# wnmusic/simpleFE

Hardware: AMD Instinct MI355X
Metric: complex-float32 MS/s through 256-tap blkconv FIR; % of HBM roofline (higher is better)
Workload: dtype f32

## Files before the change

simplefe_amd/build.py:

```python
import glob
import json
import os
import subprocess
import sys

HERE = os.path.dirname(os.path.abspath(__file__))
CSRC = os.path.join(HERE, "csrc")
LIB = os.path.join(HERE, "libsfe_dsp.so")
LIB_DIAG = os.path.join(HERE, "libsfe_dsp_diag.so")
ARCH = "gfx950"
EXACT_SOURCES = ("polyphase.hip", "util.hip", "chan.hip", "combine.hip", "ddc.hip")
TICKET_SOURCES = ("fir_fft.hip", "poly_fft.hip")
HOST_SOURCES = ("api.hip", "api_plans.hip", "api_fir.hip", "api_rs.hip", "api_pipe.hip", "api_chan.hip", "api_combine.hip", "api_ddc.hip",
                "group.hip", "host.h")


def sources(diag=False):
    return sorted(glob.glob(os.path.join(CSRC, "*.hip"))) + (sorted(glob.glob(os.path.join(CSRC, "diag", "*.hip"))) if diag else [])


def _deps():
    return sources(diag=True) + glob.glob(os.path.join(CSRC, "*.h")) + glob.glob(os.path.join(CSRC, "diag", "*.inc")) + glob.glob(
        os.path.join(os.path.dirname(HERE), "include", "*.h"))


KERNEL_FILES = {"fir": ("fir_fft.hip", "fft16.h", "common.h"), "resample": ("poly_fft.hip", "fft16.h", "common.h"),
                "decimate": ("polyphase.hip", "common.h"), "chan": ("chan.hip", "fft16.h", "common.h"),
                "combine": ("combine.hip", "fft16.h", "common.h"), "ddc": ("ddc.hip", "common.h")}


def csrc_hash(kind=None):
    import hashlib
    import re
    h = hashlib.sha256()
    paths = sorted(glob.glob(os.path.join(CSRC, "*.hip")) + glob.glob(os.path.join(CSRC, "*.h")))
    if kind is not None:
        paths = [p for p in paths if os.path.basename(p) in KERNEL_FILES[kind]]
    for p in paths:
        if os.path.basename(p) in HOST_SOURCES:
            continue
        h.update(os.path.basename(p).encode() + b"\0")
        depth, skip_at = 0, None
        for line in open(p, errors="replace"):
            code = re.sub(r"\s+", " ", re.sub(r"//.*$", "", line)).strip()
            if code.startswith("#if"):
                depth += 1
                if skip_at is None and re.match(r"#ifdef SFE_DIAG\b", code):
                    skip_at = depth
                    continue
            elif code.startswith("#else") and skip_at == depth:
                skip_at = -depth
                continue
            elif code.startswith("#endif"):
                closing = depth
                depth -= 1
                if skip_at is not None and abs(skip_at) == closing:
                    skip_at = None
                    continue
            if skip_at is not None and skip_at > 0:
                continue
            if code:
                h.update(code.encode() + b"\n")
        h.update(b"\0")
    return h.hexdigest()


def needs_build(lib=LIB):
    if not os.path.exists(lib):
        return True
    t = os.path.getmtime(lib)
    return any(os.path.getmtime(p) > t for p in _deps())


def parse_resources(text):
    import re
    out, cur = {}, None
    for line in text.splitlines():
        m = re.search(r"remark:\s+Function Name: (\S+)", line)
        if m:
            cur = out.setdefault(m.group(1), {})
            continue
        m = re.search(r"remark:\s+(TotalSGPRs|VGPRs|AGPRs|ScratchSize \[bytes/lane\]|Occupancy \[waves/SIMD\]|SGPRs Spill|VGPRs Spill|"
                      r"LDS Size \[bytes/block\]): (\d+)", line)
        if m and cur is not None:
            cur[m.group(1).split(" [")[0]] = int(m.group(2))
    if out:
        names = list(out)
        try:
            dem = subprocess.run(["c++filt"], input="\n".join(names), capture_output=True, text=True).stdout.splitlines()
        except OSError:
            dem = []
        if len(dem) == len(names):
            out = {d: out[n] for d, n in zip(dem, names)}
    return out


FIR_TEMPLATE_ARGS = "IN_C OUT_C IN_U8 PAIR OUT_TX10 DMA DIAG ACC WP HCH".split()


def fir_kernel_flags(name):
    import re
    m = re.search(r"fir_fft4096_kernel<(.*?)>\(", name)
    if not m:
        return None
    vals = [a.strip() for a in m.group(1).split(",")]
    return {k: (v == "true" if v in ("true", "false") else int(v)) for k, v in zip(FIR_TEMPLATE_ARGS, vals)}


def check_resources(res):
# ... 83 lines not shown
```

simplefe_amd/csrc/diag/fir_fft_diag.inc:

```
template <int WAVES>
__global__ __launch_bounds__(256, WAVES) void fir_copy_pattern_kernel(FirFftArgs a)
{
    const unsigned t = threadIdx.x;
    const char *in_c = static_cast<const char *>(a.in) + (size_t)blockIdx.y * a.in_stride * 8;
    char *out_c = static_cast<char *>(a.out) + (size_t)blockIdx.y * a.out_stride * 8;
    const int row0 = a.hl >> 8;
    for (long long blk = blockIdx.x; blk < a.nblk; blk += gridDim.x) {
        const long long base = blk * a.advance - a.hl;
        if (base < 0 || base + FFT_N > a.n) continue;
        v2f v[16];
#pragma unroll
        for (int r = 0; r < 16; r++) v[r] = load_sample<true>(in_c + (base + 256 * r) * 8, t);
#pragma unroll
        for (int r = 0; r < 16; r++)
            if (r >= row0) reinterpret_cast<v2f *>(out_c + (base + 256 * r) * 8)[t] = v[r];
    }
}


template <int WAVES>
__global__ __launch_bounds__(256, WAVES) void fir_copy_pattern16_kernel(FirFftArgs a)
{
    const unsigned t = threadIdx.x;
    const char *in_c = static_cast<const char *>(a.in) + (size_t)blockIdx.y * a.in_stride * 8;
    char *out_c = static_cast<char *>(a.out) + (size_t)blockIdx.y * a.out_stride * 8;
    const int row0 = a.hl >> 8;
    const unsigned half = t >> 7, col2 = t & 127;
    for (long long blk = blockIdx.x; blk < a.nblk; blk += gridDim.x) {
        const long long base = blk * a.advance - a.hl;
        if (base < 0 || base + FFT_N > a.n) continue;
        v4f v[8];
#pragma unroll
        for (int j = 0; j < 8; j++)
            v[j] = reinterpret_cast<const v4f *>(in_c + (base + 256 * (2 * j)) * 8)[col2 + 128 * half];
#pragma unroll
        for (int j = 0; j < 8; j++)
            if (2 * j + (int)half >= row0)
                reinterpret_cast<v4f *>(out_c + (base + 256 * (2 * j)) * 8)[col2 + 128 * half] = v[j];
    }
}

#define FIR_TRACE_WGS 163840
__device__ unsigned long long g_fir_trace[5 * FIR_TRACE_WGS];
__device__ unsigned long long g_fir_tdone[FIR_TRACE_WGS];
__device__ unsigned long long g_fir_tclk[FIR_TRACE_WGS];
__device__ int g_fir_gate;
__device__ int g_fir_order;

template <int WAVES, bool TICKET, bool BAR = false, bool TRACE = false>
__global__ __launch_bounds__(256, WAVES) void fir_copy_pattern_nt_kernel(FirFftArgs a)
{
    __shared__ unsigned s_next;
    const unsigned t = threadIdx.x;
    const unsigned long long t_start = TRACE ? wall_clock64() : 0ull;
    const int gate = TRACE ? g_fir_gate : 0;
    const int order = TRACE ? g_fir_order : 0;
    unsigned n_done = 0;
    const unsigned wg_lin = blockIdx.x + blockIdx.y * gridDim.x;
    auto leave = [&]() {
        if (TRACE && t == 0 && wg_lin < FIR_TRACE_WGS) {
            unsigned long long *r = g_fir_trace + 5ull * wg_lin;
            r[0] = t_start; r[1] = wall_clock64(); r[2] = n_done;
            r[3] = __builtin_amdgcn_s_getreg(20 | (3 << 11));
            r[4] = __builtin_amdgcn_s_getreg(4 | (31 << 11));
        }
    };
    const int row0 = a.hl >> 8;
    const unsigned nblk32 = (unsigned)a.nblk;
    const unsigned tg = a.tgroups, grp = blockIdx.x % tg;
    unsigned *const my_ticket = a.ticket + 32u * grp;
    const unsigned last_draw = (a.total > grp ? (a.total - grp + tg - 1u) / tg : 0u) + (gridDim.x - grp + tg - 1u) / tg - 1u;
    auto draw = [&]() -> unsigned {
        const unsigned c = __hip_atomic_fetch_add(my_ticket, 1u, __ATOMIC_RELAXED, __HIP_MEMORY_SCOPE_AGENT);
        if (c == last_draw) __hip_atomic_store(my_ticket, 0u, __ATOMIC_RELAXED, __HIP_MEMORY_SCOPE_AGENT);
        const unsigned long long k = (unsigned long long)c * tg + grp;
        return k < a.total ? (unsigned)k : 0xFFFFFFFFu;
    };
    unsigned kt = 0;
    long long blk = blockIdx.x;
    int ch = TICKET ? 0 : blockIdx.y;
    if (TICKET) {
        if (t == 0) s_next = draw();
        lds_barrier();
        kt = __builtin_amdgcn_readfirstlane(s_next);
        lds_barrier();
    }
    for (;;) {
        if (TICKET) {
            if (kt >= a.total) break;
            ch = (int)(kt / nblk32);
            blk = kt - (unsigned)ch * nblk32;
        } else if (blk >= a.nblk) break;
        const char *in_c = static_cast<const char *>(a.in) + (size_t)ch * a.in_stride * 8;
        char *out_c = static_cast<char *>(a.out) + (size_t)ch * a.out_stride * 8;
        long long pblk = blk;
        if (order == 1) pblk = a.nblk - 1 - blk;
        else if (order == 2) pblk = (long long)(((unsigned long long)blk * 48271ull) % (unsigned long long)a.nblk);
        const long long base = pblk * a.advance - a.hl;
        unsigned drawn = 0;
        if (TICKET && t == 0) drawn = draw();
        if (base >= 0 && base + FFT_N <= a.n) {
            v2f v[16];
            if (gate) while (((wall_clock64() >> gate) & 1ull) != 0ull) __builtin_amdgcn_s_sleep(1);
#pragma unroll
            for (int r = 0; r < 16; r++)
                v[r] = __builtin_nontemporal_load(reinterpret_cast<const v2f *>(in_c + (base + 256 * r) * 8) + t);
            if (BAR) { asm volatile("s_waitcnt vmcnt(0)" ::: "memory"); lds_barrier(); lds_barrier(); }
            if (gate) {
                asm volatile("s_waitcnt vmcnt(0)" ::: "memory");
                while (((wall_clock64() >> gate) & 1ull) != 1ull) __builtin_amdgcn_s_sleep(1);
            }
#pragma unroll
            for (int r = 0; r < 16; r++)
                if (r >= row0) __builtin_nontemporal_store(v[r], reinterpret_cast<v2f *>(out_c + (base + 256 * r) * 8) + t);
            if (TRACE && t == 0 && v[15].x != 1.2345e38f) {
                const unsigned long long lin = (unsigned long long)ch * nblk32 + (unsigned long long)blk;
                if (lin < FIR_TRACE_WGS) { g_fir_tdone[lin] = wall_clock64(); g_fir_tclk[lin] = clock64(); }
            }
        }
        n_done++;
        if (TICKET) {
            if (t == 0) s_next = drawn;
            lds_barrier();
            kt = __builtin_amdgcn_readfirstlane(s_next);
            lds_barrier();
        } else blk += gridDim.x;
// ... 153 lines not shown
```

simplefe_amd/csrc/diag/fir_fft_launch_diag.inc:

```
    if (ev && in_complex && out_complex && !in_u8 && !out_tx10) {
#define SFE_NEW(DM, DG, WPV) SFE_K(true, true, false, false, false, DM, DG, false, WPV)
#define SFE_NEW_DG(DM, WPV) do { if (diag == 1) SFE_NEW(DM, 1, WPV); else if (diag == 2) SFE_NEW(DM, 2, WPV); \
                                else if (diag == 3) SFE_NEW(DM, 3, WPV); else SFE_NEW(DM, 0, WPV); } while (0)
        bool done = true;
        const bool traced = (ev[0] == 'e' || ev[0] == 'E') && (getenv("SFE_FIR_TRACE") || getenv("SFE_FIR_ORDER") || getenv("SFE_FIR_GATE"));
        if (traced) {
            const int order = getenv("SFE_FIR_ORDER") ? atoi(getenv("SFE_FIR_ORDER")) : 0;
            SFE_HIP(hipMemcpyToSymbolAsync(HIP_SYMBOL(g_fir_order), &order, sizeof order, 0, hipMemcpyHostToDevice, s));
            const int gate = getenv("SFE_FIR_GATE") ? atoi(getenv("SFE_FIR_GATE")) : 0;
            SFE_HIP(hipMemcpyToSymbolAsync(HIP_SYMBOL(g_fir_gate), &gate, sizeof gate, 0, hipMemcpyHostToDevice, s));
        }
        if (ev[0] == 'c') hipLaunchKernelGGL((fir_copy_pattern_kernel<4>), grid2, block, 0, s, a);
        else if (ev[0] == 'd') hipLaunchKernelGGL((fir_copy_pattern16_kernel<4>), grid2, block, 0, s, a);
        else if (ev[0] == 'e' && traced) hipLaunchKernelGGL((fir_copy_pattern_nt_kernel<4, false, false, true>), grid2, block, 0, s, a);
        else if (ev[0] == 'E' && traced) hipLaunchKernelGGL((fir_copy_pattern_nt_kernel<4, true, false, true>), grid, block, 0, s, a);
        else if (ev[0] == 'e') hipLaunchKernelGGL((fir_copy_pattern_nt_kernel<4, false>), grid2, block, 0, s, a);
        else if (ev[0] == 'E') hipLaunchKernelGGL((fir_copy_pattern_nt_kernel<4, true>), grid, block, 0, s, a);
        else if (ev[0] == 'b') hipLaunchKernelGGL((fir_copy_pattern_nt_kernel<4, false, true>), grid2, block, 0, s, a);
        else if (ev[0] == 'g') hipLaunchKernelGGL((fir_copy_pattern_dma_kernel<4, true>), grid2, block, 0, s, a);
        else if (ev[0] == 'G') hipLaunchKernelGGL((fir_copy_pattern_dma_kernel<4, false>), grid2, block, 0, s, a);
        else if (ev[0] == 'q' || ev[0] == 'Q') {
            const int delay = getenv("SFE_FIR_DELAY") ? atoi(getenv("SFE_FIR_DELAY")) : 0;
            SFE_HIP(hipMemcpyToSymbolAsync(HIP_SYMBOL(g_fir_delay), &delay, sizeof delay, 0, hipMemcpyHostToDevice, s));
            if (ev[0] == 'q') hipLaunchKernelGGL((fir_copy_pattern_dma2_kernel<2, true>), grid2, block, 0, s, a);
            else hipLaunchKernelGGL((fir_copy_pattern_dma2_kernel<4, false>), grid2, block, 0, s, a);
        }
        else if (ev[0] == 'p') hipLaunchKernelGGL((fir_copy_pattern_pipe_kernel<4>), grid2, block, 0, s, a);
        else if (ev[0] == 'T') SFE_NEW_DG(false, false);
        else if (ev[0] == 'X') SFE_NEW_DG(true, false);
        else if (ev[0] == 'W') SFE_NEW_DG(true, true);
        else if (ev[0] == 'y') SFE_NEW(true, 8, false);
        else if (ev[0] == 'u') SFE_NEW(false, 8, false);
        else if (ev[0] == 'L') SFE_NEW(false, 16, false);
        else if (ev[0] == 'M') SFE_NEW(false, 32, false);
        else if (ev[0] == 'N') SFE_NEW(false, 48, false);
        else if (ev[0] == 'l') SFE_NEW(true, 16, false);
        else if (ev[0] == 'n') SFE_NEW(true, 48, false);
        else if (ev[0] == 'x') SFE_NEW(true, 4, false);
        else if (ev[0] == 't') SFE_NEW(false, 4, false);
        else if (ev[0] == 'w') SFE_NEW(true, 4, true);
        else done = false;
#undef SFE_NEW
#undef SFE_NEW_DG
        if (done) {
            SFE_HIP(hipGetLastError());
            if (const char *tp = getenv("SFE_FIR_TRACE")) {
                if (traced) {
                    const size_t nwg = (ev[0] == 'E' ? (size_t)grid.x : (size_t)grid2.x * grid2.y);
                    const size_t cnt = 5 * (nwg < FIR_TRACE_WGS ? nwg : FIR_TRACE_WGS);
                    unsigned long long *h = (unsigned long long *)malloc(cnt * 8);
                    SFE_HIP(hipStreamSynchronize(s));
                    SFE_HIP(hipMemcpyFromSymbol(h, HIP_SYMBOL(g_fir_trace), cnt * 8));
                    if (FILE *f = fopen(tp, "wb")) { fwrite(h, 8, cnt, f); fclose(f); }
                    free(h);
                    const size_t nt = a.total < FIR_TRACE_WGS ? a.total : FIR_TRACE_WGS;
                    h = (unsigned long long *)malloc(nt * 8);
                    SFE_HIP(hipMemcpyFromSymbol(h, HIP_SYMBOL(g_fir_tdone), nt * 8));
                    char tp2[512];
                    snprintf(tp2, sizeof tp2, "%s.done", tp);
                    if (FILE *f = fopen(tp2, "wb")) { fwrite(h, 8, nt, f); fclose(f); }
                    SFE_HIP(hipMemcpyFromSymbol(h, HIP_SYMBOL(g_fir_tclk), nt * 8));
                    snprintf(tp2, sizeof tp2, "%s.clk", tp);
                    if (FILE *f = fopen(tp2, "wb")) { fwrite(h, 8, nt, f); fclose(f); }
                    free(h);
                }
            }
            return SFE_OK;
        }
    }
```

simplefe_amd/csrc/fir_fft.hip:

```cpp
#include <stdint.h>
#include <stdlib.h>

#include "common.h"
#include "fft16.h"

namespace sfe {
namespace {

template <bool IN_C, bool IN_U8 = false>
__device__ __forceinline__ v2f load_sample(const void *p, unsigned lane)
{
    if constexpr (IN_U8) {
        if constexpr (IN_C) {
            const unsigned w = __builtin_nontemporal_load(reinterpret_cast<const unsigned short *>(p) + lane);
            return (v2f){u8_to_f32(w & 0xFFu), u8_to_f32(w >> 8)};
        } else {
            return (v2f){u8_to_f32(__builtin_nontemporal_load(reinterpret_cast<const unsigned char *>(p) + lane)), 0.0f};
        }
    }
    if constexpr (IN_C) return __builtin_nontemporal_load(reinterpret_cast<const v2f *>(p) + lane);
    else return (v2f){__builtin_nontemporal_load(reinterpret_cast<const float *>(p) + lane), 0.0f};
}

template <int K>
__device__ __forceinline__ unsigned quad_lane(unsigned v)
{
    return (unsigned)__builtin_amdgcn_update_dpp(0, (int)v, K | (K << 2) | (K << 4) | (K << 6), 0xF, 0xF, true);
}
__device__ __forceinline__ unsigned quad_odd(unsigned v)
{
    return (unsigned)__builtin_amdgcn_update_dpp(0, (int)v, 1 | (1 << 2) | (3 << 4) | (3 << 6), 0xF, 0xF, true);
}

__device__ __forceinline__ void store_group(unsigned char *d, unsigned u0, unsigned u1, unsigned u2, unsigned u3)
{
    const unsigned w = ((u0 >> 8) | ((u1 >> 8) << 2) | ((u2 >> 8) << 4) | ((u3 >> 8) << 6)) | ((u0 & 0xFFu) << 8) |
                       ((u1 & 0xFFu) << 16) | ((u2 & 0xFFu) << 24);
    __builtin_memcpy(d, &w, 4);
    d[4] = (unsigned char)u3;
}

#ifdef SFE_DIAG
__device__ unsigned long long g_fir_clk[4];
#define SFE_FIR_STAMP(i)                                                                   \
    do {                                                                                   \
        if (blockIdx.x == 0 && blockIdx.y == 0 && threadIdx.x == 0) {                      \
            g_fir_clk[i] = __builtin_amdgcn_s_memtime();                                   \
            g_fir_clk[(i) + 1] = __builtin_amdgcn_s_memrealtime();                         \
        }                                                                                  \
    } while (0)
#else
#define SFE_FIR_STAMP(i) do { } while (0)
#endif

template <bool IN_C, bool OUT_C, bool IN_U8 = false, bool PAIR = false, bool OUT_TX10 = false, bool DMA = false, int DIAG = 0,
          bool ACC = false, bool WP = false, bool HCH = false>
__global__ __launch_bounds__(256, 4) void fir_fft4096_kernel(FirFftArgs a)
{
    static_assert(!WP || DMA, "the wave-private layout exists for the LDS-DMA path");
    static_assert(!ACC || (!OUT_TX10 && !DMA), "accumulating launches write float32 through the plain store path");
    static_assert(!DMA || (IN_C && !IN_U8 && !PAIR), "LDS-DMA input: complex float32, padded layout");
    constexpr bool INTERLEAVE = (DIAG & 8) != 0;
    constexpr bool NOMID = (DIAG & 16) != 0, NORECON = (DIAG & 32) != 0;
    auto tw2f = [](v2f x, v2f q, v2f p) -> v2f { return NORECON ? cmul(x, q) : cmul2(x, q, p); };
    auto tw2i = [](v2f x, v2f q, v2f p) -> v2f { return NORECON ? cmul_conj(x, q) : cmul2_conj(x, q, p); };
    __shared__ v2f lds[WP ? 4 * WP_REGION : FFT_ROWS * LDS_K2_STRIDE];
    __shared__ unsigned s_next;
    const unsigned t = threadIdx.x;
    SFE_FIR_STAMP(0);
    int ch = 0;
    const unsigned lo = t & 15, hi = t >> 4;
    const unsigned base_a = WP ? (t >> 6) * WP_REGION + (t & 63u) : t;
    const unsigned base_b = hi * LDS_K2_STRIDE + lo;
    const unsigned base_c = hi * LDS_K2_STRIDE + lo * LDS_K1_STRIDE;
    const unsigned base_w = (hi & 7u) * WP_PITCH + (hi >> 3) * 64u + lo;
    auto row_a = [](int r) -> unsigned { return WP ? (unsigned)((r & 7) * WP_PITCH + (r >> 3) * 64) : (unsigned)(r * LDS_K2_STRIDE); };
    auto cell_b1 = [&](int a1) -> unsigned {
        if (WP) return base_w + (unsigned)((a1 >> 2) * WP_REGION + 16 * (a1 & 3));
        return base_b + 16u * a1;
    };
    auto cell_b2 = [&](int a1) -> unsigned { return base_b + (unsigned)LDS_K1_STRIDE * a1; };
    auto cell_c = [&](int n0) -> unsigned { return base_c + n0; };

    constexpr int ISZ = IN_U8 ? (IN_C ? 2 : 1) : (IN_C ? 8 : 4);
    const char *in_c, *hist_c;
    char *out_c;
    auto in_of = [&](int c) -> const char * { return static_cast<const char *>(a.in) + (size_t)c * a.in_stride * ISZ; };
    v2f hreg[16];
    auto load_spectrum = [&](int c) {
        if constexpr (HCH) {
#pragma unroll
            for (int k = 0; k < 16; k++) {
                hreg[k] = (a.hs + (size_t)c * a.hs_stride + k * 256)[threadIdx.x];
                asm volatile("" : "+v"(hreg[k]));
            }
        }
    };
    auto set_channel = [&](int c) {
        in_c = in_of(c);
        out_c = static_cast<char *>(a.out) + (OUT_TX10 ? (size_t)c * (a.out_stride * (OUT_C ? 2 : 1) / 4) * 5 : (size_t)c * a.out_stride * (OUT_C ? 8 : 4));
        hist_c = static_cast<const char *>(a.hist) + (size_t)c * a.hist_len * (IN_C ? 8 : 4);
    };
    load_spectrum(ch);
    set_channel(ch);

    v2f p1[4], q1[4], p2[4], q2[4];
#pragma unroll
    for (int k = 1; k < 4; k++) {
        p1[k] = a.tw1[k * 256 + t];
        q1[k] = a.tw1[(k + 3) * 256 + t];
        p2[k] = a.tw2[k * 16 + lo];
        q2[k] = a.tw2[(k + 3) * 16 + lo];
    }

    const int row0 = a.hl >> 8;
    auto carry_history = [&]() {
        char *ho = static_cast<char *>(a.hist_out) + (size_t)ch * a.hist_len * (IN_C ? 8 : 4);
        for (int r = 0; r < (a.hist_len >> 8); r++) {
            const v2f s = load_sample<IN_C, IN_U8>(in_c + (a.n - a.hist_len + 256 * r) * ISZ, t);
            if constexpr (IN_C) reinterpret_cast<v2f *>(ho)[256 * r + t] = s;
            else reinterpret_cast<float *>(ho)[256 * r + t] = s.x;
        }
    };
    const unsigned tg = a.tgroups, grp = blockIdx.x % tg;
    unsigned *const my_ticket = a.ticket + 32u * grp;
    const unsigned Q = 1u << a.tqs, row = tg << a.tqs, rem = a.total % row;
    const bool by_channel = HCH && a.ch_groups;
    const unsigned mine = by_channel ? (a.total / (unsigned)a.nblk / tg) * (unsigned)a.nblk
                                     : (a.total / row << a.tqs) + (rem > grp * Q ? (rem - grp * Q < Q ? rem - grp * Q : Q) : 0u);
    const unsigned last_draw = mine + (gridDim.x - grp + tg - 1u) / tg - 1u;
    const bool few = a.total <= gridDim.x;
    auto draw_issue = [&]() -> unsigned {
        if (few) return 0u;
        return __hip_atomic_fetch_add(my_ticket, 1u, __ATOMIC_RELAXED, __HIP_MEMORY_SCOPE_AGENT);
    };
    auto draw_finish = [&](unsigned c) -> unsigned {
        if (few) return 0xFFFFFFFFu;
        if (c == last_draw) __hip_atomic_store(my_ticket, 0u, __ATOMIC_RELAXED, __HIP_MEMORY_SCOPE_AGENT);
        if (by_channel) {
            if (c >= mine) return 0xFFFFFFFFu;
            const unsigned i = c / (unsigned)a.nblk;
            return (grp + tg * i) * (unsigned)a.nblk + (c - i * (unsigned)a.nblk);
        }
        const unsigned long long k = (((unsigned long long)(c >> a.tqs) * tg + grp) << a.tqs) + (c & (Q - 1u));
        return k < a.total ? (unsigned)k : 0xFFFFFFFFu;
    };
    auto draw = [&]() -> unsigned { return draw_finish(draw_issue()); };
    const unsigned nblk32 = (unsigned)a.nblk;
    if (!HCH) {
#pragma unroll
        for (int k = 0; k < 16; k++) {
            hreg[k] = (a.hs + k * 256)[t];
            asm volatile("" : "+v"(hreg[k]));
        }
    }

    auto load_rows = [&](v2f (&x)[16], long long blk) {
        constexpr int ESZ = IN_C ? 8 : 4;
        if constexpr (PAIR) {
            const long long baseA = 2 * blk * a.advance - a.hl - a.shift, baseB = baseA + a.advance;
            if constexpr (IN_U8) {
                if (baseA >= 0 && baseB + FFT_N <= a.n && (reinterpret_cast<uintptr_t>(in_c) & 15u) == 0) {
                    typedef unsigned v4u __attribute__((ext_vector_type(4)));
                    const v4u rA = __builtin_nontemporal_load(reinterpret_cast<const v4u *>(in_c + baseA) + t);
                    const v4u rB = __builtin_nontemporal_load(reinterpret_cast<const v4u *>(in_c + baseB) + t);
                    v4u *raw = reinterpret_cast<v4u *>(lds);
                    raw[t] = rA;
                    raw[256u + t] = rB;
                    lds_barrier();
                    const unsigned char *rs = reinterpret_cast<const unsigned char *>(lds);
#pragma unroll
                    for (int r = 0; r < 16; r++) x[r] = (v2f){u8_to_f32(rs[256 * r + t]), u8_to_f32(rs[4096 + 256 * r + t])};
                    lds_barrier();
                    return;
                }
            }
            if (baseA >= 0 && baseB + FFT_N <= a.n) {
#pragma unroll
                for (int r = 0; r < 16; r++)
                    x[r] = (v2f){load_sample<false, IN_U8>(in_c + (baseA + 256 * r) * ISZ, t).x,
                                 load_sample<false, IN_U8>(in_c + (baseB + 256 * r) * ISZ, t).x};
            } else {
#pragma unroll
                for (int r = 0; r < 16; r++) {
                    float p[2];
#pragma unroll
                    for (int q = 0; q < 2; q++) {
                        const long long row = (q ? baseB : baseA) + 256 * r;
                        if (row + (long long)t < 0) p[q] = load_sample<false>(hist_c + (a.hist_len + row) * ESZ, t).x;
                        else if (row + (long long)t < a.n) p[q] = load_sample<false, IN_U8>(in_c + row * ISZ, t).x;
                        else p[q] = 0.0f;
                    }
                    x[r] = (v2f){p[0], p[1]};
                }
            }
            return;
        }
        const long long base = blk * a.advance - a.hl - a.shift;
        if constexpr (DIAG & 1) {
            unsigned u = t + ((unsigned)blk << 12);
            asm volatile("" : "+v"(u));
#pragma unroll
            for (int r = 0; r < 16; r++) x[r] = (v2f){__builtin_bit_cast(float, 0x3f000000u | ((u + 256u * r) & 0x7fffffu)), 0.25f};
            return;
        }
        if constexpr (IN_U8 && IN_C) {
            if (base >= 0 && base + FFT_N <= a.n && (reinterpret_cast<uintptr_t>(in_c) & 15u) == 0) {
                typedef unsigned v4u __attribute__((ext_vector_type(4)));
                const v4u *src = reinterpret_cast<const v4u *>(in_c + base * 2);
                const v4u r0 = __builtin_nontemporal_load(src + t), r1 = __builtin_nontemporal_load(src + 256u + t);
                v4u *raw = reinterpret_cast<v4u *>(lds);
                raw[t] = r0;
                raw[256u + t] = r1;
                lds_barrier();
                const unsigned short *rs = reinterpret_cast<const unsigned short *>(lds);
#pragma unroll
                for (int r = 0; r < 16; r++) {
                    const unsigned w = rs[256 * r + t];
                    x[r] = (v2f){u8_to_f32(w & 0xFFu), u8_to_f32(w >> 8)};
                }
                lds_barrier();
                return;
            }
        }
        if (base >= 0 && base + FFT_N <= a.n) {
#pragma unroll
            for (int r = 0; r < 16; r++) {
                if (IN_C && !IN_U8 && (r == 0 || r == 15) && ((a.halo_keep >> r) & 1u))
                    x[r] = reinterpret_cast<const v2f *>(in_c + (base + 256 * r) * ISZ)[t];
                else
                    x[r] = load_sample<IN_C, IN_U8>(in_c + (base + 256 * r) * ISZ, t);
            }
        } else {
#pragma unroll
            for (int r = 0; r < 16; r++) {
                const long long row = base + 256 * r;
                if (row + (long long)t < 0) x[r] = load_sample<IN_C>(hist_c + (a.hist_len + row) * ESZ, t);
                else if (row + (long long)t < a.n) x[r] = load_sample<IN_C, IN_U8>(in_c + row * ISZ, t);
                else x[r] = (v2f){0.0f, 0.0f};
            }
        }
    };

    const unsigned lds_base = (unsigned)(size_t)(__attribute__((address_space(3))) v2f *)lds;
    const unsigned wv = __builtin_amdgcn_readfirstlane(t >> 6), lane16 = (t & 63u) * 16u;
    const unsigned lane_wp = ((t >> 5) & 1u) * (8u * 256u * 8u) + (t & 31u) * 16u;
    auto interior = [&](long long blk) -> bool {
        if constexpr (DIAG & 1) return false;
        const long long base = blk * a.advance - a.hl - a.shift;
        return base >= 0 && base + FFT_N <= a.n;
    };
    auto dma_rows = [&](const char *chan, long long blk) {
        const char *g = chan + (blk * a.advance - a.hl - a.shift) * 8;
#pragma unroll
        for (int p = 0; p < 8; p++) {
            unsigned dst, off;
            const char *gp;
            if constexpr (WP) {
                dst = lds_base + (wv * WP_REGION + (unsigned)p * WP_PITCH) * 8u;
                gp = g + ((unsigned)p * 256u + 64u * wv) * 8u;
                off = lane_wp;
            } else {
                const unsigned row = 4u * wv + (p >> 1), half = p & 1;
                dst = lds_base + (row * LDS_K2_STRIDE + half * 128u) * 8u;
                gp = g + (row * 256u + half * 128u) * 8u;
                off = lane16;
            }
            unsigned keep;
            const bool shared_row = WP ? (((a.halo_keep >> (unsigned)p) | (a.halo_keep >> (unsigned)(p + 8))) & 1u) != 0
                                       : ((a.halo_keep >> (4u * wv + (unsigned)(p >> 1))) & 1u) != 0;
            if (shared_row)
                asm volatile("s_mov_b32 %0, m0\n\ts_mov_b32 m0, %3\n\ts_nop 0\n\tglobal_load_lds_dwordx4 %1, %2\n\ts_mov_b32 m0, %0"
                             : "=&s"(keep) : "v"(off), "s"(gp), "s"(dst) : "memory");
            else
                asm volatile("s_mov_b32 %0, m0\n\ts_mov_b32 m0, %3\n\ts_nop 0\n\tglobal_load_lds_dwordx4 %1, %2 nt\n\ts_mov_b32 m0, %0"
                             : "=&s"(keep) : "v"(off), "s"(gp), "s"(dst) : "memory");
        }
    };

    v2f nx[16];
    long long blk;
    unsigned kt_next = 0;
    {
        if (t == 0) s_next = few ? blockIdx.x : draw();
        lds_barrier();
        const unsigned kt = __builtin_amdgcn_readfirstlane(s_next);
        if (kt >= a.total) return;
        ch = (int)(kt / nblk32);
        blk = kt - (unsigned)ch * nblk32;
        load_spectrum(ch);
        set_channel(ch);
    }
    bool landed = false;
    bool counted = false;
    if (DMA && interior(blk)) {
        dma_rows(in_c, blk);
        landed = true;
    }
    for (;;) {
        v2f v[16];
        if (a.hist_out && blk == 0) carry_history();
        if (DMA && landed) {
            if (counted) asm volatile("s_waitcnt vmcnt(15)" ::: "memory");
            else asm volatile("s_waitcnt vmcnt(0)" ::: "memory");
            if (!WP) lds_barrier();
#pragma unroll
            for (int r = 0; r < 16; r++) nx[r] = lds[base_a + row_a(r)];
        } else load_rows(nx, blk);
        dft16<-1>(nx);
#pragma unroll
        for (int k = 0; k < 16; k++) {
            v2f x = nx[P16(k)];
            if ((k >> 2) && (k & 3)) x = tw2f(x, q1[k >> 2], p1[k & 3]);
            else if (k >> 2) x = cmul(x, q1[k >> 2]);
            else if (k & 3) x = cmul(x, p1[k & 3]);
            lds[base_a + row_a(k)] = x;
        }
        lds_barrier();
        unsigned drawn = 0;
        if (t == 0) drawn = draw_issue();
#pragma unroll
        for (int r = 0; r < 16; r++) v[r] = lds[cell_b1(r)];
        dft16<-1>(v);
        if (!NOMID) lds_barrier();
        v2f wmid[16];
#pragma unroll
        for (int k = 0; k < 16; k++) {
            v2f x = v[P16(k)];
            if ((k >> 2) && (k & 3)) x = tw2f(x, q2[k >> 2], p2[k & 3]);
            else if (k >> 2) x = cmul(x, q2[k >> 2]);
            else if (k & 3) x = cmul(x, p2[k & 3]);
            if constexpr (NOMID) wmid[k] = x;
            else lds[cell_b2(k)] = x;
        }
        if (!NOMID) lds_barrier();
#pragma unroll
        for (int r = 0; r < 16; r++) {
            if constexpr (NOMID) v[r] = wmid[r];
            else v[r] = lds[cell_c(r)];
        }
        dft16<-1>(v);
        {
#pragma unroll
            for (int k = 0; k < 16; k++) v[P16(k)] = cmul(v[P16(k)], hreg[k]);
            dft16_rev<+1>(v);
#pragma unroll
            for (int k = 0; k < 16; k++) {
                if constexpr (NOMID) wmid[k] = v[k];
                else lds[cell_c(k)] = v[k];
            }
        }
        asm volatile("" : "+v"(drawn));
        if (t == 0) s_next = draw_finish(drawn);
        lds_barrier();
        kt_next = __builtin_amdgcn_readfirstlane(s_next);
        const bool more = kt_next < a.total;
        const int nch = (int)(kt_next / nblk32);
        const long long nb = kt_next - (unsigned)nch * nblk32;
        if (HCH && more && nch != ch) load_spectrum(nch);
#pragma unroll
        for (int r = 0; r < 16; r++) {
            v2f x;
            if constexpr (NOMID) x = wmid[r];
            else x = lds[cell_b2(r)];
            if ((r >> 2) && (r & 3)) x = tw2i(x, q2[r >> 2], p2[r & 3]);
            else if (r >> 2) x = cmul_conj(x, q2[r >> 2]);
            else if (r & 3) x = cmul_conj(x, p2[r & 3]);
// ... 100 lines not shown
            if constexpr (OUT_TX10 && OUT_C) {
            typedef int v1i;
            char *const wb = out_c + (obase >> 1) * 5;
            const unsigned lo = __builtin_amdgcn_readfirstlane((unsigned)reinterpret_cast<uintptr_t>(wb));
            const unsigned hi = __builtin_amdgcn_readfirstlane((unsigned)(reinterpret_cast<uintptr_t>(wb) >> 32));
            const __amdgpu_buffer_rsrc_t rs = __builtin_amdgcn_make_buffer_rsrc(
                reinterpret_cast<void *>(((uintptr_t)hi << 32) | lo), 0, (FFT_N / 2) * 5, 0x00020000);
            int sel = (t & 1u) ? (int)0x7FFF0000 : (int)((t >> 1) * 5u);
            asm volatile("" : "+v"(sel));
#pragma unroll
            for (int r = 1; r < 16; r++) {
                const v2f y = v[P16(r)];
                const unsigned u0 = (unsigned)((int)(short)(int)(y.x * 511.0f) + 512) & 0x3FFu;
                const unsigned u1 = (unsigned)((int)(short)(int)(y.y * 511.0f) + 512) & 0x3FFu;
                const unsigned u2 = quad_odd(u0), u3 = quad_odd(u1);
                const unsigned w = ((u0 >> 8) | ((u1 >> 8) << 2) | ((u2 >> 8) << 4) | ((u3 >> 8) << 6)) | ((u0 & 0xFFu) << 8) |
                                   ((u1 & 0xFFu) << 16) | ((u2 & 0xFFu) << 24);
                const int up = 640 * r;
                __builtin_amdgcn_raw_buffer_store_b32((v1i)w, rs, sel + (up & 2047), up & ~2047, 0);
                __builtin_amdgcn_raw_buffer_store_b8((unsigned char)u3, rs, sel + (up & 2047) + 4, up & ~2047, 0);
            }
            }
        } else if (plain_rows) {
#pragma unroll
            for (int b = 0; b < 4; b++) {
                if constexpr (INTERLEAVE) dft16_tail<+1>(v, b);
#pragma unroll
            for (int c = 0; c < 4; c++) {
                const int r = b + 4 * c;
                if (r == 0) continue;
                if constexpr (DIAG & 2) continue;
                v2f y = v[P16(r)];
                char *rp = DMA ? obase_p + (voff + (unsigned)(256 * r * OSZ)) : out_c + (obase + 256 * r) * OSZ + (size_t)t * OSZ;
                if constexpr (OUT_C) {
                    if constexpr (ACC) y += *reinterpret_cast<const v2f *>(rp);
                    __builtin_nontemporal_store(y, reinterpret_cast<v2f *>(rp));
                } else {
                    if constexpr (ACC) y.x += *reinterpret_cast<const float *>(rp);
                    __builtin_nontemporal_store(y.x, reinterpret_cast<float *>(rp));
                }
            }
            }
        } else {
        if constexpr (INTERLEAVE) {
#pragma unroll
            for (int b = 0; b < 4; b++) dft16_tail<+1>(v, b);
        }
#pragma unroll
        for (int r = 0; r < 16; r++) {
            const long long orow = obase + 256 * r;
            if constexpr (OUT_TX10 && OUT_C) {
                if (r < row0) continue;
                const v2f y = v[P16(r)];
                const unsigned u0 = (unsigned)((int)(short)(int)(y.x * 511.0f) + 512) & 0x3FFu;
                const unsigned u1 = (unsigned)((int)(short)(int)(y.y * 511.0f) + 512) & 0x3FFu;
                const unsigned u2 = quad_odd(u0), u3 = quad_odd(u1);
                if ((t & 1u) == 0 && orow + (long long)t + 1 < a.n) {
                    unsigned char *d = reinterpret_cast<unsigned char *>(out_c) + ((orow + (long long)t) >> 1) * 5;
                    store_group(d, u0, u1, u2, u3);
                }
                continue;
            }
            if constexpr (DIAG & 2) continue;
            if (r >= row0 && (whole || orow + (long long)t < a.n)) {
                v2f y = v[P16(r)];
                char *rp = DMA ? obase_p + (voff + (unsigned)(256 * r * OSZ)) : out_c + orow * OSZ + (size_t)t * OSZ;
                if constexpr (OUT_C) {
                    if constexpr (ACC) y += *reinterpret_cast<const v2f *>(rp);
                    __builtin_nontemporal_store(y, reinterpret_cast<v2f *>(rp));
                } else {
                    if constexpr (ACC) y.x += *reinterpret_cast<const float *>(rp);
                    __builtin_nontemporal_store(y.x, reinterpret_cast<float *>(rp));
                }
            }
        }
        }
        if constexpr (DIAG & 2) {
            v2f acc = v[0];
#pragma unroll
            for (int r = 1; r < 16; r++) acc += v[r];
            if (acc.x == 1.2345e38f) reinterpret_cast<v2f *>(out_c)[t] = acc;
        }
        }
        if (!more) break;
        blk = nb;
        if (nch != ch) {
            ch = nch;
            set_channel(ch);
        }
    }
    SFE_FIR_STAMP(2);
}


#ifdef SFE_DIAG
#include "diag/fir_fft_diag.inc"
#endif

}

#ifdef SFE_DIAG
extern "C" int sfe_dsp_diag_fir_clock(double *mhz, double *ms)
{
    unsigned long long c[4];
    SFE_HIP(hipMemcpyFromSymbol(c, HIP_SYMBOL(g_fir_clk), sizeof c));
    const double dr = (double)(c[3] - c[1]);
    if (mhz) *mhz = dr > 0 ? (double)(c[2] - c[0]) / dr * 100.0 : 0.0;
    if (ms) *ms = dr / 1e5;
    return SFE_OK;
}
#endif

bool fir_fft_has_variants(const FirFftArgs &a, int in_complex, int out_complex, int in_u8, int out_tx10, int n_channels, int accumulate)
{
    const bool dma_ok = (reinterpret_cast<uintptr_t>(a.in) & 15u) == 0 && (n_channels == 1 || (a.in_stride & 1) == 0);
    return in_complex && out_complex && !in_u8 && !out_tx10 && !accumulate && dma_ok;
}

int launch_fir_fft(const FirFftArgs &a0, int in_complex, int out_complex, int in_u8, int out_tx10, int n_channels,
                   hipStream_t s, int accumulate)
{
    FirFftArgs a = a0;
    if (a.nblk <= 0) return SFE_OK;
    if (a.hist_len < a.hl + a.shift || (a.hist_len & 255) || (a.shift & 255) || ((accumulate || a.shift) && out_tx10)) {
        set_error("fir_fft: bad partition arguments (hist_len=%d hl=%d shift=%d)", a.hist_len, a.hl, a.shift);
        return SFE_EINVAL;
    }
    if (a.hl <= 0 || (a.hl & 255) || a.hl >= FFT_N || a.advance != FFT_N - a.hl) {
        set_error("fir_fft: bad overlap rows (hl=%d advance=%d)", a.hl, a.advance);
        return SFE_EINVAL;
    }
    if (in_complex && !out_complex) {
        set_error("fir_fft: complex input with real output is not a defined combination");
        return SFE_EINVAL;
    }
    if ((out_tx10 || in_u8) && in_complex != out_complex) {
        set_error("fir_fft: wire-format input/output is built for real->real and complex->complex streams");
        return SFE_EINVAL;
    }
    int wg_per_cu = 8;
    const bool pair = !in_complex && !out_complex;
    const bool dma_ok = (reinterpret_cast<uintptr_t>(a.in) & 15u) == 0 && (n_channels == 1 || (a.in_stride & 1) == 0);
    const int var = !dma_ok ? FIR_VAR_REG : (a.variant == FIR_VAR_DMA || a.variant == FIR_VAR_WP ? a.variant : FIR_VAR_REG);
#ifdef SFE_DIAG
    const char *ev = getenv("SFE_FIR_VARIANT");
    const int diag = getenv("SFE_FIR_DIAG") ? atoi(getenv("SFE_FIR_DIAG")) & 3 : 0;
    if (const char *e = getenv("SFE_FIR_WG_PER_CU")) wg_per_cu = atoi(e) > 0 ? atoi(e) : wg_per_cu;
#endif
    long long nb = pair ? (a.nblk + 1) / 2 : a.nblk;
    a.nblk = nb;
    const long long total = nb * n_channels;
    const int cus = device_cu_count();
    long long gt = total < (long long)cus * wg_per_cu ? total : (long long)cus * wg_per_cu;
    if (total + gt >= 0xFFFFFFFFLL || !a.ticket) {
        set_error("fir_fft: %lld transforms in one launch exceed the ticket counter", total);
        return SFE_ERANGE;
    }
    a.total = (unsigned)total;
    a.tgroups = FIR_TICKET_GROUPS;
#ifdef SFE_DIAG
    if (const char *e = getenv("SFE_FIR_TGROUPS")) a.tgroups = atoi(e) >= 1 && atoi(e) <= FIR_TICKET_GROUPS_MAX ? atoi(e) : a.tgroups;
#endif
    if ((long long)a.tgroups > gt) a.tgroups = (unsigned)gt;
    a.ch_groups = a.hs_stride != 0 && a.tgroups == FIR_TICKET_GROUPS && n_channels >= (int)a.tgroups && n_channels % (int)a.tgroups == 0;
#ifdef SFE_DIAG
    if (const char *e = getenv("SFE_FIR_CH_GROUPS")) a.ch_groups = a.ch_groups && atoi(e) != 0;
#endif
    a.tqs = 3;
    a.halo_keep = 0x8001u;
#ifdef SFE_DIAG
    if (const char *e = getenv("SFE_FIR_HALO_KEEP")) a.halo_keep = (unsigned)strtoul(e, nullptr, 0);
    if (const char *e = getenv("SFE_FIR_TQS")) a.tqs = atoi(e) >= 0 && atoi(e) <= 8 ? (unsigned)atoi(e) : 0u;
#endif
    const dim3 grid((unsigned)gt), block(256);
#define SFE_K(...) hipLaunchKernelGGL((fir_fft4096_kernel<__VA_ARGS__>), grid, block, 0, s, a)
#ifdef SFE_DIAG
    long long gx = nb;
    const long long cap = ((long long)cus * wg_per_cu + n_channels - 1) / n_channels;
    if (gx > cap) gx = cap < 1 ? 1 : cap;
    const dim3 grid2((unsigned)gx, (unsigned)n_channels);
#include "diag/fir_fft_launch_diag.inc"
#endif
    if (a.hs_stride) {
        if (!in_complex || !out_complex || in_u8 || out_tx10) {
            set_error("fir_fft: per-channel taps are built for complex float32 streams");
            return SFE_EINVAL;
        }
        if (accumulate) SFE_K(true, true, false, false, false, false, 0, true, false, true);
        else if (var != FIR_VAR_REG) SFE_K(true, true, false, false, false, true, 0, false, false, true);
        else SFE_K(true, true, false, false, false, false, 0, false, false, true);
    } else if (accumulate) {
        if (in_complex) {
            if (in_u8) SFE_K(true, true, true, false, false, false, 0, true);
            else SFE_K(true, true, false, false, false, false, 0, true);
        } else if (out_complex) {
            SFE_K(false, true, false, false, false, false, 0, true);
        } else {
            if (in_u8) SFE_K(false, false, true, true, false, false, 0, true);
            else SFE_K(false, false, false, true, false, false, 0, true);
        }
    } else if (in_complex) {
        if (in_u8 && out_tx10) SFE_K(true, true, true, false, true);
        else if (out_tx10) SFE_K(true, true, false, false, true);
        else if (in_u8) SFE_K(true, true, true);
        else if (var == FIR_VAR_DMA) SFE_K(true, true, false, false, false, true);
        else if (var == FIR_VAR_WP) SFE_K(true, true, false, false, false, true, 0, false, true);
        else SFE_K(true, true);
    } else if (out_complex) {
        SFE_K(false, true);
    } else {
        if (in_u8 && out_tx10) SFE_K(false, false, true, true, true);
        else if (out_tx10) SFE_K(false, false, false, true, true);
        else if (in_u8) SFE_K(false, false, true, true);
        else SFE_K(false, false, false, true);
    }
#undef SFE_K
    SFE_HIP(hipGetLastError());
    return SFE_OK;
}

}
```

Measured before the change: 338,400.

## Add work stealing across ticket groups in FIR block scheduler

Moves ticket logic into a shared header. Workgroups that exhaust their own group's ticket counter now steal blocks from other groups' counters, tracking exhausted groups in a shared bitmask. Counter reset moves to a last-exiter protocol using exit and out counters in place of the old last-draw store. The goal is to balance load across ticket groups and cut tail imbalance, at the cost of extra atomics on the draw path and more bookkeeping per workgroup. Diagnostic tracing hooks are added but compile away in the default build.

```diff
diff --git a/simplefe_amd/build.py b/simplefe_amd/build.py
--- a/simplefe_amd/build.py
+++ b/simplefe_amd/build.py
@@ -24,7 +24,7 @@
         os.path.join(os.path.dirname(HERE), "include", "*.h"))
 
 
-KERNEL_FILES = {"fir": ("fir_fft.hip", "fft16.h", "common.h"), "resample": ("poly_fft.hip", "fft16.h", "common.h"),
+KERNEL_FILES = {"fir": ("fir_fft.hip", "fft16.h", "common.h", "ticket.h"), "resample": ("poly_fft.hip", "fft16.h", "common.h"),
                 "decimate": ("polyphase.hip", "common.h"), "chan": ("chan.hip", "fft16.h", "common.h"),
                 "combine": ("combine.hip", "fft16.h", "common.h"), "ddc": ("ddc.hip", "common.h")}
 
diff --git a/simplefe_amd/csrc/diag/fir_fft_diag.inc b/simplefe_amd/csrc/diag/fir_fft_diag.inc
--- a/simplefe_amd/csrc/diag/fir_fft_diag.inc
+++ b/simplefe_amd/csrc/diag/fir_fft_diag.inc
@@ -40,8 +40,6 @@
     }
 }
 
-#define FIR_TRACE_WGS 163840
-__device__ unsigned long long g_fir_trace[5 * FIR_TRACE_WGS];
 __device__ unsigned long long g_fir_tdone[FIR_TRACE_WGS];
 __device__ unsigned long long g_fir_tclk[FIR_TRACE_WGS];
 __device__ int g_fir_gate;
diff --git a/simplefe_amd/csrc/diag/fir_fft_launch_diag.inc b/simplefe_amd/csrc/diag/fir_fft_launch_diag.inc
--- a/simplefe_amd/csrc/diag/fir_fft_launch_diag.inc
+++ b/simplefe_amd/csrc/diag/fir_fft_launch_diag.inc
@@ -9,6 +9,11 @@
             SFE_HIP(hipMemcpyToSymbolAsync(HIP_SYMBOL(g_fir_order), &order, sizeof order, 0, hipMemcpyHostToDevice, s));
             const int gate = getenv("SFE_FIR_GATE") ? atoi(getenv("SFE_FIR_GATE")) : 0;
             SFE_HIP(hipMemcpyToSymbolAsync(HIP_SYMBOL(g_fir_gate), &gate, sizeof gate, 0, hipMemcpyHostToDevice, s));
+        }
+        const bool ptraced = (ev[0] == 'T' || ev[0] == 'X' || ev[0] == 'W') && diag == 0 && getenv("SFE_FIR_TRACE");
+        if (ev[0] == 'T' || ev[0] == 'X' || ev[0] == 'W') {
+            const int on = ptraced ? 1 : 0;
+            SFE_HIP(hipMemcpyToSymbolAsync(HIP_SYMBOL(g_fir_ptrace), &on, sizeof on, 0, hipMemcpyHostToDevice, s));
         }
         if (ev[0] == 'c') hipLaunchKernelGGL((fir_copy_pattern_kernel<4>), grid2, block, 0, s, a);
         else if (ev[0] == 'd') hipLaunchKernelGGL((fir_copy_pattern16_kernel<4>), grid2, block, 0, s, a);
@@ -45,6 +50,14 @@
         if (done) {
             SFE_HIP(hipGetLastError());
             if (const char *tp = getenv("SFE_FIR_TRACE")) {
+                if (ptraced) {
+                    const size_t cnt = 5 * ((size_t)grid.x < FIR_TRACE_WGS ? (size_t)grid.x : FIR_TRACE_WGS);
+                    unsigned long long *h = (unsigned long long *)malloc(cnt * 8);
+                    SFE_HIP(hipStreamSynchronize(s));
+                    SFE_HIP(hipMemcpyFromSymbol(h, HIP_SYMBOL(g_fir_trace), cnt * 8));
+                    if (FILE *f = fopen(tp, "wb")) { fwrite(h, 8, cnt, f); fclose(f); }
+                    free(h);
+                }
                 if (traced) {
                     const size_t nwg = (ev[0] == 'E' ? (size_t)grid.x : (size_t)grid2.x * grid2.y);
                     const size_t cnt = 5 * (nwg < FIR_TRACE_WGS ? nwg : FIR_TRACE_WGS);
diff --git a/simplefe_amd/csrc/fir_fft.hip b/simplefe_amd/csrc/fir_fft.hip
--- a/simplefe_amd/csrc/fir_fft.hip
+++ b/simplefe_amd/csrc/fir_fft.hip
@@ -3,6 +3,7 @@
 
 #include "common.h"
 #include "fft16.h"
+#include "ticket.h"
 
 namespace sfe {
 namespace {
@@ -49,8 +50,39 @@
             g_fir_clk[(i) + 1] = __builtin_amdgcn_s_memrealtime();                         \
         }                                                                                  \
     } while (0)
+#define FIR_TRACE_WGS 163840
+__device__ unsigned long long g_fir_trace[5 * FIR_TRACE_WGS];
+__device__ int g_fir_ptrace;
+__device__ unsigned long long g_fir_steal_force;
+#define SFE_FIR_TRACE_BEGIN()                                                              \
+    __shared__ unsigned s_tr[2];                                                           \
+    do {                                                                                   \
+        if (threadIdx.x == 0) {                                                            \
+            s_tr[0] = s_tr[1] = 0;                                                         \
+            if (DIAG == 0 && blockIdx.x < FIR_TRACE_WGS && g_fir_ptrace) {                  \
+                g_fir_trace[5ull * blockIdx.x] = wall_clock64();                           \
+                g_fir_trace[5ull * blockIdx.x + 1] = 0;                                    \
+            }                                                                              \
+        }                                                                                  \
+    } while (0)
+#define SFE_FIR_TRACE_COUNT() do { if (threadIdx.x == 0) s_tr[0]++; } while (0)
+#define SFE_FIR_TRACE_STOLEN() do { s_tr[1]++; } while (0)
+#define SFE_FIR_TRACE_LEAVE()                                                              \
+    do {                                                                                   \
+        if (DIAG == 0 && threadIdx.x == 0 && blockIdx.x < FIR_TRACE_WGS && g_fir_ptrace) { \
+            unsigned long long *r = g_fir_trace + 5ull * blockIdx.x;                       \
+            r[1] = wall_clock64();                                                         \
+            r[2] = s_tr[0] | (unsigned long long)s_tr[1] << 32;                            \
+            r[3] = __builtin_amdgcn_s_getreg(20 | (3 << 11));                              \
+            r[4] = __builtin_amdgcn_s_getreg(4 | (31 << 11));                              \
+        }                                                                                  \
+    } while (0)
 #else
 #define SFE_FIR_STAMP(i) do { } while (0)
+#define SFE_FIR_TRACE_BEGIN() do { } while (0)
+#define SFE_FIR_TRACE_COUNT() do { } while (0)
+#define SFE_FIR_TRACE_STOLEN() do { } while (0)
+#define SFE_FIR_TRACE_LEAVE() do { } while (0)
 #endif
 
 template <bool IN_C, bool OUT_C, bool IN_U8 = false, bool PAIR = false, bool OUT_TX10 = false, bool DMA = false, int DIAG = 0,
@@ -68,6 +100,7 @@
     __shared__ unsigned s_next;
     const unsigned t = threadIdx.x;
     SFE_FIR_STAMP(0);
+    SFE_FIR_TRACE_BEGIN();
     int ch = 0;
     const unsigned lo = t & 15, hi = t >> 4;
     const unsigned base_a = WP ? (t >> 6) * WP_REGION + (t & 63u) : t;
@@ -123,29 +156,51 @@
         }
     };
     const unsigned tg = a.tgroups, grp = blockIdx.x % tg;
-    unsigned *const my_ticket = a.ticket + 32u * grp;
-    const unsigned Q = 1u << a.tqs, row = tg << a.tqs, rem = a.total % row;
     const bool by_channel = HCH && a.ch_groups;
-    const unsigned mine = by_channel ? (a.total / (unsigned)a.nblk / tg) * (unsigned)a.nblk
-                                     : (a.total / row << a.tqs) + (rem > grp * Q ? (rem - grp * Q < Q ? rem - grp * Q : Q) : 0u);
-    const unsigned last_draw = mine + (gridDim.x - grp + tg - 1u) / tg - 1u;
+    const TicketMap tmap = {a.total, tg, a.tqs, by_channel ? (unsigned)a.nblk : 0u};
+    const unsigned mine = ticket_share(tmap, grp);
     const bool few = a.total <= gridDim.x;
+    __shared__ unsigned s_cur;
+    auto fetch_add = [&](unsigned *word) -> unsigned { return __hip_atomic_fetch_add(word, 1u, __ATOMIC_RELAXED, __HIP_MEMORY_SCOPE_AGENT); };
+    auto fresh_args = [&]() -> const __attribute__((address_space(4))) FirFftArgs * {
+        auto *ap = (const __attribute__((address_space(4))) FirFftArgs *)__builtin_amdgcn_kernarg_segment_ptr();
+        asm volatile("" : "+s"(ap));
+        return ap;
+    };
+    auto fresh_map = [&](const __attribute__((address_space(4))) FirFftArgs *ap) -> TicketMap {
+        return {ap->total, ap->tgroups, ap->tqs, by_channel ? (unsigned)ap->nblk : 0u};
+    };
+    auto steal = [&](unsigned cur, bool seen) -> unsigned {
+        const auto *ap = fresh_args();
+        const unsigned k = ticket_steal(ap->ticket, fresh_map(ap), blockIdx.x, gridDim.x, cur, seen, &s_cur);
+        if (k != TICKET_NONE) SFE_FIR_TRACE_STOLEN();
+        return k;
+    };
     auto draw_issue = [&]() -> unsigned {
         if (few) return 0u;
-        return __hip_atomic_fetch_add(my_ticket, 1u, __ATOMIC_RELAXED, __HIP_MEMORY_SCOPE_AGENT);
+        return fetch_add(a.ticket + TICKET_LINE * s_cur);
     };
     auto draw_finish = [&](unsigned c) -> unsigned {
-        if (few) return 0xFFFFFFFFu;
-        if (c == last_draw) __hip_atomic_store(my_ticket, 0u, __ATOMIC_RELAXED, __HIP_MEMORY_SCOPE_AGENT);
-        if (by_channel) {
-            if (c >= mine) return 0xFFFFFFFFu;
-            const unsigned i = c / (unsigned)a.nblk;
-            return (grp + tg * i) * (unsigned)a.nblk + (c - i * (unsigned)a.nblk);
-        }
-        const unsigned long long k = (((unsigned long long)(c >> a.tqs) * tg + grp) << a.tqs) + (c & (Q - 1u));
-        return k < a.total ? (unsigned)k : 0xFFFFFFFFu;
-    };
-    auto draw = [&]() -> unsigned { return draw_finish(draw_issue()); };
+        if (few) return TICKET_NONE;
+        const unsigned cur = s_cur;
+        if (cur == grp) {
+            if (c < mine) return ticket_transform(tmap, grp, c);
+        } else {
+            const TicketMap m = fresh_map(fresh_args());
+            if (c < ticket_share(m, cur)) {
+                SFE_FIR_TRACE_STOLEN();
+                return ticket_transform(m, cur, c);
+            }
+        }
+        return steal(cur, true);
+    };
+    auto draw_first = [&]() -> unsigned {
+        s_cur = grp;
+#ifdef SFE_DIAG
+        if (tg > 1 && ((g_fir_steal_force >> grp) & 1ull)) return steal(grp, false);
+#endif
+        return draw_finish(draw_issue());
+    };
     const unsigned nblk32 = (unsigned)a.nblk;
     if (!HCH) {
 #pragma unroll
@@ -282,7 +337,7 @@
     long long blk;
     unsigned kt_next = 0;
     {
-        if (t == 0) s_next = few ? blockIdx.x : draw();
+        if (t == 0) s_next = few ? blockIdx.x : draw_first();
         lds_barrier();
         const unsigned kt = __builtin_amdgcn_readfirstlane(s_next);
         if (kt >= a.total) return;
@@ -549,6 +604,7 @@
             if (acc.x == 1.2345e38f) reinterpret_cast<v2f *>(out_c)[t] = acc;
         }
         }
+        SFE_FIR_TRACE_COUNT();
         if (!more) break;
         blk = nb;
         if (nch != ch) {
@@ -557,6 +613,7 @@
         }
     }
     SFE_FIR_STAMP(2);
+    SFE_FIR_TRACE_LEAVE();
 }
 
 
@@ -646,6 +703,15 @@
     const long long cap = ((long long)cus * wg_per_cu + n_channels - 1) / n_channels;
     if (gx > cap) gx = cap < 1 ? 1 : cap;
     const dim3 grid2((unsigned)gx, (unsigned)n_channels);
+    {
+        static unsigned long long force_sent = 0;
+        const char *e = getenv("SFE_FIR_STEAL_FORCE");
+        const unsigned long long force = e ? strtoull(e, nullptr, 0) : 0ull;
+        if (force != force_sent) {
+            SFE_HIP(hipMemcpyToSymbolAsync(HIP_SYMBOL(g_fir_steal_force), &force, sizeof force, 0, hipMemcpyHostToDevice, s));
+            force_sent = force;
+        }
+    }
 #include "diag/fir_fft_launch_diag.inc"
 #endif
     if (a.hs_stride) {
diff --git a/simplefe_amd/csrc/ticket.h b/simplefe_amd/csrc/ticket.h
--- /dev/null
+++ b/simplefe_amd/csrc/ticket.h
@@ -0,0 +1,85 @@
+#pragma once
+
+#if defined(__HIPCC__) || defined(__CUDACC__)
+#define SFE_TK_HD __host__ __device__ __forceinline__
+#else
+#define SFE_TK_HD inline
+#endif
+
+namespace sfe {
+
+constexpr unsigned TICKET_LINE = 32;
+constexpr unsigned TICKET_EXIT_WORD = 16;
+constexpr unsigned TICKET_MASK_LINE = 63;
+constexpr unsigned TICKET_MASK_WORD = TICKET_MASK_LINE * TICKET_LINE + 8;
+constexpr unsigned TICKET_OUT_WORD = TICKET_MASK_LINE * TICKET_LINE + 12;
+constexpr unsigned TICKET_NONE = 0xFFFFFFFFu;
+
+struct TicketMap {
+    unsigned total;
+    unsigned tg;
+    unsigned tqs;
+    unsigned chn;
+};
+
+SFE_TK_HD unsigned ticket_share(const TicketMap &m, unsigned g)
+{
+    if (m.chn) return (m.total / m.chn / m.tg) * m.chn;
+    const unsigned Q = 1u << m.tqs, row = m.tg << m.tqs, rem = m.total % row;
+    return (m.total / row << m.tqs) + (rem > g * Q ? (rem - g * Q < Q ? rem - g * Q : Q) : 0u);
+}
+
+SFE_TK_HD unsigned ticket_transform(const TicketMap &m, unsigned g, unsigned c)
+{
+    if (m.chn) {
+        const unsigned i = c / m.chn;
+        return (g + m.tg * i) * m.chn + (c - i * m.chn);
+    }
+    return ((((c >> m.tqs) * m.tg) + g) << m.tqs) + (c & ((1u << m.tqs) - 1u));
+}
+
+SFE_TK_HD unsigned ticket_group_size(unsigned grid, unsigned tg, unsigned g) { return (grid - g + tg - 1u) / tg; }
+
+SFE_TK_HD unsigned ticket_next_victim(unsigned grp, unsigned cur, unsigned tg, unsigned mask)
+{
+    for (unsigned v = (cur + tg - grp) % tg + 1u; v < tg; v++) {
+        const unsigned g = (grp + v) % tg;
+        if (g >= 32u || !((mask >> g) & 1u)) return g;
+    }
+    return tg;
+}
+
+#if defined(__HIPCC__)
+__device__ inline unsigned ticket_steal(unsigned *tk, const TicketMap &m, unsigned block, unsigned grid, unsigned cur, bool seen, unsigned *s_cur)
+{
+    auto fetch_add = [](unsigned *w) -> unsigned { return __hip_atomic_fetch_add(w, 1u, __ATOMIC_RELAXED, __HIP_MEMORY_SCOPE_AGENT); };
+    unsigned *const mask = tk + TICKET_MASK_WORD;
+    auto mark = [&](unsigned g) -> unsigned {
+        if (g >= 32u) return __hip_atomic_load(mask, __ATOMIC_RELAXED, __HIP_MEMORY_SCOPE_AGENT);
+        return __hip_atomic_fetch_or(mask, 1u << g, __ATOMIC_RELAXED, __HIP_MEMORY_SCOPE_AGENT) | 1u << g;
+    };
+    const unsigned tg = m.tg, grp = block % tg;
+    unsigned seen_mask = seen ? mark(cur) : __hip_atomic_load(mask, __ATOMIC_RELAXED, __HIP_MEMORY_SCOPE_AGENT);
+    for (unsigned i = 1; i < tg; i++) {
+        cur = ticket_next_victim(grp, cur, tg, seen_mask);
+        if (cur >= tg) break;
+        const unsigned c = fetch_add(tk + TICKET_LINE * cur);
+        if (c < ticket_share(m, cur)) {
+            *s_cur = cur;
+            return ticket_transform(m, cur, c);
+        }
+        seen_mask = mark(cur);
+    }
+    if (fetch_add(tk + TICKET_LINE * grp + TICKET_EXIT_WORD) == ticket_group_size(grid, tg, grp) - 1u && fetch_add(tk + TICKET_OUT_WORD) == tg - 1u) {
+        for (unsigned g = 0; g < tg; g++) {
+            __hip_atomic_store(tk + TICKET_LINE * g, 0u, __ATOMIC_RELAXED, __HIP_MEMORY_SCOPE_AGENT);
+            __hip_atomic_store(tk + TICKET_LINE * g + TICKET_EXIT_WORD, 0u, __ATOMIC_RELAXED, __HIP_MEMORY_SCOPE_AGENT);
+        }
+        __hip_atomic_store(mask, 0u, __ATOMIC_RELAXED, __HIP_MEMORY_SCOPE_AGENT);
+        __hip_atomic_store(tk + TICKET_OUT_WORD, 0u, __ATOMIC_RELAXED, __HIP_MEMORY_SCOPE_AGENT);
+    }
+    return TICKET_NONE;
+}
+#endif
+
+}
```

Result: no change. 338,500 (median of 3 runs) (+0.0%).
